# asharakeh/pod_compare

Measured on AMD Instinct MI355X. Metric: images/sec (BayesOD+MC-dropout, 1280x720), higher is better.
Workload: dtype f32 (convolutions: every fp32 product from 2-way f16 splits of the power-of-two-scaled fp32 operands, 3 partial products, fp32 accumulate; closer to fp64 than the fp32 MFMA: profiles/r05_f16_split_numerics.txt)

## Files before the change

include/pod_mi355x.h:

```cpp
#ifndef POD_MI355X_H
#define POD_MI355X_H

#include <stddef.h>
#include <stdint.h>

#ifdef __cplusplus
extern "C" {
#endif

#define POD_ABI_VERSION 18
#define POD_MAX_LEVELS 8
#define POD_MAX_CLASSES 16
#define POD_MAX_RUNS 64
#define POD_MAX_TOPK 2048
#define POD_MAX_PROP_SAMPLES 1024
#define POD_MAX_CLS_SAMPLES 64
#define POD_MAX_CANDIDATES 8192
#define POD_MAX_DETECTIONS 128
#define POD_COCO_MAX_IOU 16
#define POD_COCO_MAX_REC 128
#define POD_COCO_MAX_AREA 4
#define POD_COCO_MAX_MAXDET 4
#define POD_COCO_MAX_KEEP 128
#define POD_COCO_LDS_GT 64
// ... 280 lines not shown
int pod_resize_coeffs(int32_t in_size, int32_t out_size, int32_t* bounds, int32_t* coeffs);
int pod_resize_frame_u8(const uint8_t* src, int32_t in_h, int32_t in_w, int64_t row_stride, const int32_t* xbounds, const int32_t* xcoeffs,
                        int32_t xk, const int32_t* ybounds, const int32_t* ycoeffs, int32_t yk, uint8_t* dst, int32_t out_h, int32_t out_w,
                        int32_t flip_channels, pod_stream_t stream);

int pod_label_anchors(const float* anchors, int32_t R, const float* gt_boxes, const int32_t* gt_classes, const int32_t* gt_off,
                      int32_t n_images, int32_t n_gt, int32_t num_classes, float iou_low, float iou_high, int32_t* labels,
                      int32_t* matched_gt, int32_t* num_pos, uint32_t* scratch, pod_stream_t stream);

typedef struct PodLevelGrad {
    float* cls;  float* cls_var;  float* delta;  float* reg_var;
} PodLevelGrad;
int64_t pod_train_loss_partials(const PodConfig* cfg, const PodLevel* levels);
int pod_train_loss(const PodConfig* cfg, const PodLevel* levels, const PodLevelGrad* grads, const int32_t* labels,
                   const int32_t* matched_gt, const float* gt_boxes, int32_t n_gt, const float* anchors, int32_t R,
                   float alpha, float gamma, float smooth_l1_beta, const float* eps_cls, float* eps_out, const float* w,
                   double* partials, double* sums, pod_stream_t stream);

int64_t pod_conv3x3_wgrad_partials(const int32_t* level_hw, int32_t n_levels, int32_t copies, int32_t C, int32_t K, int32_t Kpad);
int pod_conv3x3_wgrad(const float* x, const float* dy, const int32_t* level_hw, int32_t n_levels, int32_t copies, int32_t C, int32_t K,
                      int32_t Kpad, const float* x_amax, const float* dy_amax, float* dW, float* db, float* partials, pod_stream_t stream);
int pod_relu_dropout_backward(const float* out, const float* d_out, float* d_z, int64_t n, float p, float* dz_amax, pod_stream_t stream);

int64_t pod_conv1x1_wgrad_partials(int64_t pixels, int32_t C, int32_t K);
int pod_conv1x1_wgrad(const float* x, const float* dy, int64_t pixels, int32_t C, int32_t K, const float* x_amax, const float* dy_amax, float* dW,
                      float* db, float* partials, pod_stream_t stream);
int pod_col2im3x3s2_cl(const float* dcols, const float* gate, const float* add, float* dx, int32_t H, int32_t W, int32_t C, float* dx_amax,
                       pod_stream_t stream);
int pod_upsample2_sum_cl(const float* d_child, int32_t h, int32_t w, const float* add, float* d_top, int32_t C, float* d_top_amax, pod_stream_t stream);


#define POD_C1_RELU 1
#define POD_C1_RESIDUAL_UP2 2
int64_t pod_conv1x1_filter_split_bytes(int32_t Cout, int32_t Cin);
int pod_conv1x1_filter_split(const float* weight, void* Ws, int32_t Cout, int32_t Cin, pod_stream_t stream);
int pod_reduce_partials(const float* partials, int32_t n_splits, int64_t split_stride, const float* bias, const float* residual, float* y,
                        int64_t n, int32_t Cout, int32_t relu, float* out_amax, pod_stream_t stream);
int pod_conv1x1_split(const float* x, float* y, const void* Ws, const float* bias, const float* residual, int32_t H_out, int32_t W_out,
                      int32_t H_in, int32_t W_in, int32_t stride, int32_t Cin, int32_t Cout, int32_t flags, int32_t n_splits, float* partials,
                      int32_t waves, const float* in_amax, float* out_amax, pod_stream_t stream);

typedef struct PodWorkspace {
    const float* anchors;
    float* mean_cls;  float* mean_cls_var;  float* mean_delta;  float* mean_reg_var;
    uint64_t* cand_keys;  int32_t* cand_count;  uint64_t* maybe_bits;
    uint64_t* sel_keys;   int32_t* sel_count;
    uint64_t* cat_keys;   int32_t* cat_level;
    float* probs_dense;
    int32_t* n_total;     int32_t* cand_anchor_idx;  int32_t* cand_level;  int32_t* cand_class;
    float* cand_score;    float* cand_probs;  float* cand_delta;  float* cand_reg_var;  float* cand_anchor;
    float* cand_run_delta;
    float* boxes;  float* cov;
    int32_t* keep;  int32_t* n_keep;  void* nms_scratch;
    float* m_boxes;  float* m_cov;  float* m_scores;  int32_t* m_classes;  float* m_probs;
    int32_t n_capacity;  int32_t reserved;
} PodWorkspace;

#define POD_MODE_STANDARD_NMS 0
#define POD_MODE_BAYES_OD 1
#define POD_MODE_ANCHOR_STATISTICS 2

int pod_run_image(const PodConfig* cfg, const PodLevel* levels, const PodWorkspace* ws, int32_t mode,
                  int32_t box_merge_mode, int32_t cls_merge_mode, int32_t image_h, int32_t image_w,
                  int32_t out_h, int32_t out_w, const PodDetections* out, pod_stream_t stream);
int pod_run_image_part(const PodConfig* cfg, const PodLevel* levels, const PodWorkspace* ws, int32_t mode,
                  int32_t box_merge_mode, int32_t cls_merge_mode, int32_t image_h, int32_t image_w,
// ... 7 lines not shown
```

pod_compare_amd/conv1x1.py:

```python
from typing import Optional

import torch

from . import amax, hip


class Conv1x1:

    def __init__(self, weight: torch.Tensor, bias: Optional[torch.Tensor], stride: int = 1):
        assert weight.is_cuda and weight.dtype == torch.float32 and weight.dim() == 4 and tuple(weight.shape[2:]) == (1, 1)
        self.K, self.C, self.stride = int(weight.shape[0]), int(weight.shape[1]), int(stride)
        if self.C % 16 or self.K % 64 or self.stride not in (1, 2):
            raise ValueError("pod_conv1x1_split: Cin %% 16 == 0, Cout %% 64 == 0, stride 1 or 2 required, got Cin=%d Cout=%d stride=%d" % (self.C, self.K, self.stride))
        self.Ws = torch.empty(2 * self.K * self.C + 8, dtype=torch.int16, device=weight.device)
        hip.check(hip.load().pod_conv1x1_filter_split(weight.detach().reshape(self.K, self.C).contiguous().data_ptr(), self.Ws.data_ptr(), self.K, self.C,
                                                      hip.current_stream()), "pod_conv1x1_filter_split")
        self.bias = None if bias is None else bias.detach().to(torch.float32).contiguous().clone()

    @staticmethod
    def eligible(conv: Optional[torch.nn.Conv2d]) -> bool:
        return (conv is not None and tuple(conv.kernel_size) == (1, 1) and tuple(conv.padding) == (0, 0) and conv.groups == 1
                and tuple(conv.dilation) == (1, 1) and conv.stride[0] == conv.stride[1] and conv.stride[0] in (1, 2)
                and conv.in_channels % 16 == 0 and conv.out_channels % 64 == 0)

    def out_hw(self, h: int, w: int):
        return ((h - 1) // self.stride + 1, (w - 1) // self.stride + 1)

    def splits_for(self, p_out: int, simds: int = 1024) -> int:
        tiles = ((p_out + 63) // 64) * (self.K // 64)
        nks = self.C // 16
        out_mb = p_out * self.K * 4 / 1e6
        step = 0.38
        best, best_t = 1, (nks // self.auto_waves(tiles, nks)) * step
        for s in (2, 4, 8, 16):
            if nks % s or nks // s < 4 or tiles * s > simds:
                continue
            t = (nks // s // self.auto_waves(tiles * s, nks // s)) * step + 3.0 + (s + 1) * out_mb / 4.0
            if t < best_t:
                best, best_t = s, t
        return best

    @staticmethod
    def auto_waves(tiles: int, per_split: int) -> int:
        waves = 1
        while waves < 4 and per_split % (waves * 4) == 0 and per_split // (waves * 2) >= 8 and tiles * waves * 2 <= 1024:
            waves *= 2
        return waves

    def __call__(self, x: torch.Tensor, h: int, w: int, relu: bool = False, residual: Optional[torch.Tensor] = None,
                 n_splits: Optional[int] = None, waves: int = 0, out: Optional[torch.Tensor] = None, residual_up2: bool = False) -> torch.Tensor:
        assert x.is_cuda and x.dtype == torch.float32 and x.is_contiguous() and tuple(x.shape) == (h * w, self.C)
        ho, wo = self.out_hw(h, w)
        y = torch.empty((ho * wo, self.K), dtype=torch.float32, device=x.device) if out is None else out
        assert y.is_contiguous() and tuple(y.shape) == (ho * wo, self.K) and y.dtype == torch.float32
        s = self.splits_for(ho * wo) if n_splits is None else int(n_splits)
        if residual is not None and residual_up2:
            hr, wr = (ho + 1) // 2, (wo + 1) // 2
            assert residual.is_contiguous() and tuple(residual.shape) == (hr * wr, self.K) and residual.dtype == torch.float32
            if s > 1:
                residual = residual.view(hr, wr, self.K).repeat_interleave(2, 0).repeat_interleave(2, 1)[:ho, :wo].reshape(ho * wo, self.K).contiguous()
                residual_up2 = False
        else:
            residual_up2 = False
        if residual is not None and not residual_up2:
            assert residual.is_contiguous() and tuple(residual.shape) == tuple(y.shape) and residual.dtype == torch.float32
        partials = torch.empty((s, ho * wo, self.K), dtype=torch.float32, device=x.device) if s > 1 else None
        hip.check(hip.load().pod_conv1x1_split(x.data_ptr(), y.data_ptr(), self.Ws.data_ptr(), hip.ptr(self.bias), hip.ptr(residual), ho, wo, h, w, self.stride,
                                               self.C, self.K, (1 if relu else 0) | (2 if residual_up2 else 0), s, hip.ptr(partials), int(waves), amax.of(x).data_ptr(), amax.produced(y).data_ptr(),
                                               hip.current_stream()), "pod_conv1x1_split")
        return y


class Stem7x7:

    def __init__(self, weight: torch.Tensor, bias: Optional[torch.Tensor]):
        assert weight.is_cuda and weight.dtype == torch.float32 and tuple(weight.shape) == (64, 3, 7, 7)
        self.Ws = torch.empty(2 * 64 * 192 + 8, dtype=torch.int16, device=weight.device)
        self._bounds = {}
        hip.check(hip.load().pod_stem7x7_filter_split(weight.detach().contiguous().data_ptr(), self.Ws.data_ptr(), hip.current_stream()), "pod_stem7x7_filter_split")
        self.bias = None if bias is None else bias.detach().to(torch.float32).contiguous().clone()

    @staticmethod
    def eligible(conv: Optional[torch.nn.Conv2d]) -> bool:
        return (conv is not None and tuple(conv.weight.shape) == (64, 3, 7, 7) and tuple(conv.stride) == (2, 2) and tuple(conv.padding) == (3, 3)
                and conv.groups == 1 and tuple(conv.dilation) == (1, 1))

    def __call__(self, x: torch.Tensor, relu: bool = True, mean: Optional[torch.Tensor] = None, std: Optional[torch.Tensor] = None,
                 padded_hw: Optional[tuple] = None):
        assert x.is_cuda and x.dtype in (torch.float32, torch.uint8) and x.is_contiguous() and x.numel() == 3 * x.shape[-2] * x.shape[-1]
        hi, wi = int(x.shape[-2]), int(x.shape[-1])
        h, w = (hi, wi) if padded_hw is None else (int(padded_hw[0]), int(padded_hw[1]))
        assert (mean is None) == (std is None) and h >= hi and w >= wi
        if mean is not None:
            assert mean.is_cuda and std.is_cuda and mean.dtype == std.dtype == torch.float32 and mean.numel() == std.numel() == 3 and mean.is_contiguous() and std.is_contiguous()
        ho, wo = (h - 1) // 2 + 1, (w - 1) // 2 + 1
        y = torch.empty((ho * wo, 64), dtype=torch.float32, device=x.device)
        bound = self._input_bound(x, mean, std)
        hip.check(hip.load().pod_stem7x7_split(x.data_ptr(), 1 if x.dtype == torch.uint8 else 0, hi, wi, hip.ptr(mean), hip.ptr(std), y.data_ptr(), self.Ws.data_ptr(),
                                               hip.ptr(self.bias), h, w, 1 if relu else 0, bound.data_ptr(), amax.produced(y).data_ptr(),
                                               hip.current_stream()), "pod_stem7x7_split")
        return y, ho, wo
# ... 53 lines not shown
```

pod_compare_amd/csrc/k13_conv1x1_split.hip:

```cpp
#include "pod_split_gemm.h"

#ifdef POD_C1_TRACE
static __device__ long long g_c1_trace[8192 * 4];
static __device__ long long g_c1_cycles[8192 * 4];
#define C1_STAMP(k)                                                                                   \
    do {                                                                                              \
        const unsigned wg_ = blockIdx.y * gridDim.x + blockIdx.x;                                     \
        if (threadIdx.x == 0 && wg_ < 8192) {                                                         \
            g_c1_trace[wg_ * 4 + (k)] = wall_clock64();                                               \
            g_c1_cycles[wg_ * 4 + (k)] = clock64();                                                   \
        }                                                                                             \
    } while (0)
#else
#define C1_STAMP(k)
#endif

namespace pod {

struct C1Params {
    const float* x;
    float* y;
    const uint16_t* Ws;
    const float* in_amax;
    float* out_amax;
    const float* bias;
    const float* residual;
    int32_t P_out, W_out, W_in, stride, Cin, Cout, relu;
    int32_t res_up2, W_res;
    int32_t n_pt, n_ct;
    int32_t ks_per_split;
    int64_t split_stride;
};

__global__ void __launch_bounds__(256) k_conv1x1_filter_split(const float* __restrict__ w, uint16_t* __restrict__ Ws, const float* __restrict__ amax, int32_t Cout,
                                                              int32_t Cin) {
    const int64_t t = (int64_t)blockIdx.x * blockDim.x + threadIdx.x;
    if (t >= (int64_t)Cout * (Cin / 2)) return;
    const int k = (int)(t / (Cin / 2)), c = 2 * (int)(t % (Cin / 2));
    sg_store_filter_terms(Ws, Cin >> 4, k, c, w[(int64_t)k * Cin + c], w[(int64_t)k * Cin + c + 1], amax);
}

template <int NCB>
__global__ void __launch_bounds__(64) k_conv1x1_split(const C1Params P) {
    const int lane = threadIdx.x & 63, i32 = lane & 31, h = lane >> 5;
    const int xcd = blockIdx.x & 7, wi = (int)(blockIdx.x >> 3);
    const int tp = (wi / P.n_ct) * 8 + xcd, tc = wi % P.n_ct;
    if (tp >= P.n_pt) return;
    C1_STAMP(0);
    const int nks_all = P.Cin >> 4, ks0 = (int)blockIdx.y * P.ks_per_split, nks = P.ks_per_split;
    int pout[2], pin[2];
#pragma unroll
    for (int pb = 0; pb < 2; ++pb) {
        const int p = tp * 64 + pb * 32 + i32;
        pout[pb] = p < P.P_out ? p : -1;
        const int q = p < P.P_out ? p : 0;
        if (P.stride == 1) {
            pin[pb] = q;
        } else {
            const int oy = q / P.W_out, ox = q - oy * P.W_out;
            pin[pb] = (P.stride * oy) * P.W_in + P.stride * ox;
        }
    }
    const float* __restrict__ xa[2];
#pragma unroll
// ... 97 lines not shown
__device__ __forceinline__ void c1_epilogue(const C1Params& P, float* const lds_o, f32x16 (&acc)[2][2], int tp, int tc, int lane, float sx) {
    float* __restrict__ const yo = P.y + (int64_t)blockIdx.y * P.split_stride;
    const float* __restrict__ const res = P.residual;
    const bool final_pass = P.split_stride == 0;
    const int oc = lane & 15, op = lane >> 4;
    const int gp0 = tp * 64 + op;
    const int64_t e0 = (int64_t)gp0 * P.Cout + tc * 64 + 4 * oc;
    f32x4 r[16];
    if (final_pass && res && P.res_up2) {
        int oy = gp0 / P.W_out, ox = gp0 - oy * P.W_out;
#pragma unroll
        for (int j = 0; j < 16; ++j) {
            r[j] = (gp0 + 4 * j < P.P_out) ? *reinterpret_cast<const f32x4*>(res + ((int64_t)(oy >> 1) * P.W_res + (ox >> 1)) * P.Cout + tc * 64 + 4 * oc)
                                           : f32x4{0.f, 0.f, 0.f, 0.f};
            ox += 4;
            while (ox >= P.W_out) {
                ox -= P.W_out;
                ++oy;
            }
        }
    } else if (final_pass && res) {
#pragma unroll
        for (int j = 0; j < 16; ++j) r[j] = (gp0 + 4 * j < P.P_out) ? *reinterpret_cast<const f32x4*>(res + e0 + (int64_t)(4 * j) * P.Cout) : f32x4{0.f, 0.f, 0.f, 0.f};
    }
    f32x4 b4 = f32x4{0.f, 0.f, 0.f, 0.f};
    if (final_pass && P.bias) b4 = *reinterpret_cast<const f32x4*>(P.bias + tc * 64 + 4 * oc);
    sg_line_epilogue(lds_o, acc, lane, sg_inverse_scale(sx, P.Ws, (int64_t)P.Cout * P.Cin * 2), b4, final_pass && res ? r : nullptr, final_pass && P.relu,
                     final_pass ? P.out_amax : nullptr, [&](int j, int, float*& dst) __attribute__((always_inline)) {
                         dst = yo + e0 + (int64_t)(4 * j) * P.Cout;
                         return gp0 + 4 * j < P.P_out;
                     });
}

template <int NCB, int WAVES>
__global__ void __launch_bounds__(64 * WAVES, WAVES > 1 ? 1 : 2) k_conv1x1_split_lds(const C1Params P) {
    __shared__ __attribute__((aligned(16))) float lds_all[WAVES][2][64 * 32];
    const int wave = threadIdx.x >> 6;
    float (*const lds_a)[64 * 32] = lds_all[wave];
    const int lane = threadIdx.x & 63, i32 = lane & 31, h = lane >> 5;
    const int xcd = blockIdx.x & 7, wi = (int)(blockIdx.x >> 3);
    const int tp = (wi / P.n_ct) * 8 + xcd, tc = wi % P.n_ct;
    if (tp >= P.n_pt) return;
    C1_STAMP(0);
    const int nks_all = P.Cin >> 4, nks = P.ks_per_split / WAVES, ks0 = (int)blockIdx.y * P.ks_per_split + wave * nks;
    int32_t soff[8];
#pragma unroll
    for (int j = 0; j < 8; ++j) {
        const int pl = 8 * j + (lane >> 3), p = tp * 64 + pl;
        const int q = p < P.P_out ? p : 0;
        int pin = q;
        if (P.stride != 1) {
            const int oy = q / P.W_out, ox = q - oy * P.W_out;
            pin = (P.stride * oy) * P.W_in + P.stride * ox;
        }
        soff[j] = pin * P.Cin + ks0 * 16 + 4 * ((lane & 7) ^ ((pl >> 1) & 7));
    }
    const float* __restrict__ const xg = P.x;
    const int key = (i32 >> 1) & 7;
    const uint16_t* __restrict__ const wa = P.Ws + ((int64_t)(tc * NCB) * nks_all + ks0) * SG_KS_U16 + (h * 32 + i32) * 8;
    const int64_t w_cb = (int64_t)nks_all * SG_KS_U16;
    const float sx = sg_activation_scale(P.in_amax);

    f32x16 acc[NCB][2];
#pragma unroll
    for (int cb = 0; cb < NCB; ++cb)
#pragma unroll
        for (int pb = 0; pb < 2; ++pb)
#pragma unroll
// ... 15 lines not shown
        constexpr int t = decltype(t_t)::value;
        sg_kstep<false>(acc, wf[buf], sx, [&](int pb, int i) __attribute__((always_inline)) {
            const f32x4 a = *reinterpret_cast<const f32x4*>(&lds_a[b][(pb * 32 + i32) * 32 + 4 * ((4 * t + 2 * h + (i >> 1)) ^ key)]);
            return f32x2{a[2 * (i & 1)], a[2 * (i & 1) + 1]};
        });
    };
    stage_load(0);
    load_w(sg_ic<0>{}, 0);
    load_w(sg_ic<1>{}, 1);
    stage_write(0);
    if (npairs > 1) stage_load(1);
    C1_STAMP(1);
    auto trip = [&](auto self, auto r_t, int j0) __attribute__((always_inline)) -> void {
        constexpr int R = decltype(r_t)::value;
        if constexpr (R < 6) {
            const int j = j0 + R;
            if (j < nks) {
                if (j + 2 < nks) load_w(sg_ic<(R + 2) % 3>{}, j + 2);
                const int pair = j >> 1;
                step(sg_ic<R % 3>{}, sg_ic<R & 1>{}, pair & 1);
                if constexpr ((R & 1) == 1) {
                    if (pair + 1 < npairs) {
                        stage_write((pair + 1) & 1);
                        if (pair + 2 < npairs) stage_load(pair + 2);
                    }
                }
                self(self, sg_ic<R + 1>{}, j0);
            }
        }
    };
    for (int j0 = 0; j0 < nks; j0 += 6) trip(trip, sg_ic<0>{}, j0);
    C1_STAMP(2);

    if constexpr (WAVES > 1) {
        if (wave > 0) {
            float* o = &lds_a[0][0];
#pragma unroll
            for (int cb = 0; cb < NCB; ++cb)
#pragma unroll
                for (int pb = 0; pb < 2; ++pb)
#pragma unroll
                    for (int r = 0; r < 16; ++r) o[((cb * 2 + pb) * 16 + r) * 64 + lane] = acc[cb][pb][r];
        }
        __syncthreads();
        if (wave > 0) return;
#pragma unroll
        for (int w = 1; w < WAVES; ++w) {
            const float* o = &lds_all[w][0][0];
#pragma unroll
            for (int cb = 0; cb < NCB; ++cb)
#pragma unroll
                for (int pb = 0; pb < 2; ++pb)
#pragma unroll
                    for (int r = 0; r < 16; ++r) acc[cb][pb][r] += o[((cb * 2 + pb) * 16 + r) * 64 + lane];
        }
    }
    c1_epilogue(P, &lds_a[0][0], acc, tp, tc, lane, sx);
#ifdef POD_C1_TRACE
    __builtin_amdgcn_s_waitcnt(0);
    C1_STAMP(3);
#endif
}

__global__ void __launch_bounds__(256) k_conv1x1_reduce(const float* __restrict__ partials, int32_t n_splits, int64_t split_stride, const float* __restrict__ bias,
                                                        const float* __restrict__ residual, float* __restrict__ y, int64_t n4, int32_t Cout, int32_t relu,
                                                        float* __restrict__ out_amax) {
    const int64_t stride = (int64_t)gridDim.x * blockDim.x;
// ... 1 lines not shown
    for (int64_t i = (int64_t)blockIdx.x * blockDim.x + threadIdx.x; i < n4; i += stride) {
        const f32x4 v = sg_split_sum4(partials, 4 * i, n_splits, split_stride, bias, [&](int64_t e) { return (int)(e % Cout); }, residual, relu);
        *reinterpret_cast<f32x4*>(y + 4 * i) = v;
        lmax = wino_absmax4(lmax, v);
    }
    if (out_amax) wino_publish_amax_block(out_amax, lmax);
}

}

extern "C" int64_t pod_conv1x1_filter_split_bytes(int32_t Cout, int32_t Cin) {
    if (Cout < 32 || (Cout & 31) != 0 || Cin < 16 || (Cin & 15) != 0) return 0;
    return (int64_t)Cout * Cin * 4 + 16;
}

extern "C" int pod_conv1x1_filter_split(const float* weight, void* Ws, int32_t Cout, int32_t Cin, pod_stream_t stream) {
    if (!weight || !Ws || Cout < 32 || (Cout & 31) != 0 || Cin < 16 || (Cin & 15) != 0 || !pod_aligned(16, Ws)) return POD_E_INVALID;
    const int64_t n = (int64_t)Cout * (Cin / 2);
    return pod::sg_filter_prepare(weight, (int64_t)Cout * Cin, Ws, (int64_t)Cout * Cin * 2, (hipStream_t)stream, [&](const float* amax) {
        hipLaunchKernelGGL(pod::k_conv1x1_filter_split, dim3((unsigned)((n + 255) / 256)), dim3(256), 0, (hipStream_t)stream, weight, reinterpret_cast<uint16_t*>(Ws), amax,
                           Cout, Cin);
    });
}

extern "C" int pod_conv1x1_split(const float* x, float* y, const void* Ws, const float* bias, const float* residual, int32_t H_out, int32_t W_out, int32_t H_in,
                                 int32_t W_in, int32_t stride, int32_t Cin, int32_t Cout, int32_t flags, int32_t n_splits, float* partials, int32_t waves,
                                 const float* in_amax, float* out_amax, pod_stream_t stream) {
    if (!x || !y || !Ws || !in_amax || x == y || H_out < 1 || W_out < 1 || (stride != 1 && stride != 2) || Cin < 16 || (Cin & 15) != 0 || Cout < 64 || (Cout & 63) != 0)
        return POD_E_INVALID;
    if (H_in < (H_out - 1) * stride + 1 || W_in < (W_out - 1) * stride + 1 || (stride == 1 && (H_in != H_out || W_in != W_out))) return POD_E_INVALID;
    const int64_t P_out = (int64_t)H_out * W_out;
    if (P_out * (Cout > Cin ? Cout : Cin) >= ((int64_t)1 << 31) || (int64_t)H_in * W_in * Cin >= ((int64_t)1 << 31)) return POD_E_INVALID;
    const int nks = Cin / 16;
    if (n_splits < 1 || n_splits > 16 || nks % n_splits != 0 || (n_splits > 1 && !partials)) return POD_E_INVALID;
    const int res_up2 = (flags & POD_C1_RESIDUAL_UP2) ? 1 : 0, relu = flags & POD_C1_RELU;
    if (res_up2 && (!residual || n_splits > 1)) return POD_E_INVALID;
    if (waves < 0 || waves > 4 || waves == 3) return POD_E_INVALID;
    {
        const int per_split = nks / n_splits;
        if (waves == 0) {
            const int64_t tiles = ((P_out + 63) / 64) * (Cout / 64) * n_splits;
            waves = 1;
            while (waves < 4 && per_split % (waves * 4) == 0 && per_split / (waves * 2) >= 8 && tiles * waves * 2 <= 1024) waves *= 2;
        }
        if (waves > 1 && (per_split % (2 * waves) != 0)) return POD_E_INVALID;
    }
    if (!pod_aligned(16, x, y, Ws, bias, residual, partials) || !pod_aligned(4, in_amax, out_amax)) return POD_E_INVALID;
    pod::C1Params P;
    P.x = x; P.y = n_splits > 1 ? partials : y; P.Ws = reinterpret_cast<const uint16_t*>(Ws); P.bias = bias; P.residual = residual;
    P.in_amax = in_amax; P.out_amax = out_amax;
    P.P_out = (int32_t)P_out; P.W_out = W_out; P.W_in = W_in; P.stride = stride; P.Cin = Cin; P.Cout = Cout; P.relu = relu;
    P.res_up2 = res_up2; P.W_res = (W_out + 1) / 2;
    P.n_pt = (int32_t)((P_out + 63) / 64); P.n_ct = Cout / 64;
    P.ks_per_split = nks / n_splits;
    P.split_stride = n_splits > 1 ? P_out * Cout : 0;
    const int64_t grid = 8LL * ((P.n_pt + 7) / 8) * P.n_ct;
    if (grid > 0x7FFFFFFFLL) return POD_E_INVALID;
    if ((P.ks_per_split & 1) == 0 && waves == 4)
        hipLaunchKernelGGL((pod::k_conv1x1_split_lds<2, 4>), dim3((unsigned)grid, (unsigned)n_splits), dim3(256), 0, (hipStream_t)stream, P);
    else if ((P.ks_per_split & 1) == 0 && waves == 2)
        hipLaunchKernelGGL((pod::k_conv1x1_split_lds<2, 2>), dim3((unsigned)grid, (unsigned)n_splits), dim3(128), 0, (hipStream_t)stream, P);
    else if ((P.ks_per_split & 1) == 0)
        hipLaunchKernelGGL((pod::k_conv1x1_split_lds<2, 1>), dim3((unsigned)grid, (unsigned)n_splits), dim3(64), 0, (hipStream_t)stream, P);
    else
        hipLaunchKernelGGL((pod::k_conv1x1_split<2>), dim3((unsigned)grid, (unsigned)n_splits), dim3(64), 0, (hipStream_t)stream, P);
    POD_CHECK_LAUNCH();
    if (n_splits > 1) {
        const int64_t n4 = P_out * Cout / 4;
        hipLaunchKernelGGL(pod::k_conv1x1_reduce, dim3(pod_grid_stride_blocks(n4, 2048)), dim3(256), 0, (hipStream_t)stream, partials, n_splits, P_out * Cout, bias, residual, y, n4,
                           Cout, relu, out_amax);
        POD_CHECK_LAUNCH();
    }
    return POD_OK;
}

extern "C" int pod_reduce_partials(const float* partials, int32_t n_splits, int64_t split_stride, const float* bias, const float* residual, float* y, int64_t n,
                                   int32_t Cout, int32_t relu, float* out_amax, pod_stream_t stream) {
    if (!partials || !y || n_splits < 1 || n_splits > 16 || n < 0 || (n & 3) != 0 || Cout < 4 || (Cout & 3) != 0 || n % Cout != 0) return POD_E_INVALID;
    if (n_splits > 1 && (split_stride < n || (split_stride & 3) != 0)) return POD_E_INVALID;
    if (!pod_aligned(16, partials, y, bias, residual)) return POD_E_INVALID;
    if (n == 0) return POD_OK;
    hipLaunchKernelGGL(pod::k_conv1x1_reduce, dim3(pod_grid_stride_blocks(n / 4, 4096)), dim3(256), 0, (hipStream_t)stream, partials, n_splits, split_stride, bias, residual, y, n / 4,
                       Cout, relu, out_amax);
    POD_CHECK_LAUNCH();
    return POD_OK;
}


#ifdef POD_C1_TRACE
#include <algorithm>
#include <stdio.h>
#include <vector>
extern "C" int pod_c1_trace_dump(void) {
    static long long host[8192 * 4], cyc[8192 * 4];
    if (hipDeviceSynchronize() != hipSuccess) return POD_E_LAUNCH;
    if (hipMemcpyFromSymbol(host, HIP_SYMBOL(g_c1_trace), sizeof(host)) != hipSuccess) return POD_E_LAUNCH;
    if (hipMemcpyFromSymbol(cyc, HIP_SYMBOL(g_c1_cycles), sizeof(cyc)) != hipSuccess) return POD_E_LAUNCH;
    long long t0 = 0, t_end = 0;
    std::vector<long long> start, first, loop, epi, total, mhz;
    for (int i = 0; i < 8192; ++i)
// ... 23 lines not shown
```

pod_compare_amd/csrc/pod_split_gemm.h:

```cpp
#pragma once
#include <type_traits>
#include <utility>

#include "pod_device.h"

namespace pod {

typedef float f32x16 __attribute__((ext_vector_type(16)));
typedef float f32x2 __attribute__((ext_vector_type(2)));

typedef _Float16 wino_f16x2 __attribute__((ext_vector_type(2)));
typedef _Float16 wino_f16x8 __attribute__((ext_vector_type(8)));
__device__ __forceinline__ float wino_pow2_scale(float amax, int top) {
    const int E = (int)((__float_as_uint(amax) >> 23) & 0xFFu);
    int b = 254 + top - E;
    b = b < 1 ? 1 : b > 254 ? 254 : b;
    return __uint_as_float((uint32_t)b << 23);
}
__device__ __forceinline__ float wino_pow2_inverse(float s) {
    return __uint_as_float((254u << 23) - __float_as_uint(s));
}
__device__ __forceinline__ uint32_t wino_f16_pair_scaled(float lo, float hi, float s) {
    uint32_t w;
    asm("v_fma_mixlo_f16 %0, %1, %3, 0\n\tv_fma_mixhi_f16 %0, %2, %3, 0" : "=&v"(w) : "v"(lo), "v"(hi), "s"(s));
// ... 121 lines not shown

template <typename Where>
__device__ __forceinline__ void sg_line_epilogue(float* lds, const f32x16 (&acc)[2][2], int lane, float inv1, const f32x4& b4, const f32x4* r, bool relu, float* out_amax,
                                                 Where&& where) {
    const int i32 = lane & 31, h = lane >> 5, oc = lane & 15, op = lane >> 4;
    const f32x4 inv = f32x4{inv1, inv1, inv1, inv1};
    float lmax = 0.0f;
#pragma unroll
    for (int pb = 0; pb < 2; ++pb)
#pragma unroll
        for (int cb = 0; cb < 2; ++cb)
#pragma unroll
            for (int q = 0; q < 4; ++q) {
                const int pix = 32 * pb + i32, c = 8 * cb + 2 * q + h;
                *reinterpret_cast<f32x4*>(lds + pix * 64 + 4 * (c ^ (i32 & 15))) =
                    f32x4{acc[cb][pb][4 * q], acc[cb][pb][4 * q + 1], acc[cb][pb][4 * q + 2], acc[cb][pb][4 * q + 3]};
            }
#pragma unroll
    for (int j = 0; j < 16; ++j) {
        const int pix = 4 * j + op;
        float* dst;
        const bool inside = where(j, pix, dst);
        f32x4 v = __builtin_elementwise_fma(*reinterpret_cast<const f32x4*>(lds + pix * 64 + 4 * (oc ^ (pix & 15))), inv, b4);
        if (r) v += r[j];
        if (relu) wino_relu4(v);
        if (inside) {
            *reinterpret_cast<f32x4*>(dst) = v;
            lmax = wino_absmax4(lmax, v);
        }
    }
    if (out_amax) wino_publish_amax(out_amax, lmax);
}

template <typename T>
__global__ void __launch_bounds__(256) k_sg_filter_amax(const T* __restrict__ w, int64_t n, float* __restrict__ amax) {
    float m = 0.0f;
    for (int64_t i = (int64_t)blockIdx.x * blockDim.x + threadIdx.x; i < n; i += (int64_t)gridDim.x * blockDim.x) m = fmaxf(m, fabsf(w[i]));
    wino_publish_amax1(amax, m);
}
__device__ __forceinline__ void sg_store_filter_terms(uint16_t* __restrict__ Ws, int nks, int co, int k, float lo, float hi, const float* __restrict__ amax) {
    uint32_t terms[2];
    wino_f16_split2(lo, hi, wino_pow2_scale(*amax, SG_TOP), terms);
    const int cb = co >> 5, i32 = co & 31, ks = k >> 4, h = (k >> 3) & 1, e = k & 7;
#pragma unroll
    for (int term = 0; term < 2; ++term) {
        uint16_t* d = Ws + ((((int64_t)cb * nks + ks) * 2 + term) * 2 + h) * 256 + i32 * 8 + e;
        d[0] = (uint16_t)(terms[term] & 0xFFFFu);
        d[1] = (uint16_t)(terms[term] >> 16);
    }
}
template <typename LaunchSplit>
inline int sg_filter_prepare(const float* weight, int64_t n, void* Ws, int64_t n_terms, hipStream_t stream, LaunchSplit&& launch_split) {
    float* amax = reinterpret_cast<float*>(reinterpret_cast<uint16_t*>(Ws) + n_terms);
    if (hipMemsetAsync(amax, 0, 16, stream) != hipSuccess) return POD_E_LAUNCH;
    const int64_t blocks = (n + 255) / 256;
    hipLaunchKernelGGL(k_sg_filter_amax<float>, dim3((unsigned)(blocks < 256 ? blocks : 256)), dim3(256), 0, stream, weight, n, amax);
    POD_CHECK_LAUNCH();
    launch_split(amax);
    POD_CHECK_LAUNCH();
    return POD_OK;
}

}
```

pod_compare_amd/csrc/k12_wino_conv_split.hip:

```cpp
#include "pod_wino.h"

namespace pod {

typedef uint32_t vu32x4 __attribute__((ext_vector_type(4)));
constexpr int WINO_US_BYTES = 24 * 2 * 2 * 64 * 16;
constexpr int WINO_U_TOP = 14, WINO_V_TOP = 9;
constexpr int WINO_WAIT_VM24 = 0x4078;

__global__ void __launch_bounds__(256) k_wino_filter_amax(const float* __restrict__ w, float* __restrict__ amax, int32_t K, int32_t C, int32_t Kpad) {
    const int64_t t = (int64_t)blockIdx.x * blockDim.x + threadIdx.x;
    float m = 0.0f;
    if (t < (int64_t)Kpad * C) {
        float u[4][6];
        wino_filter_values(w, (int)(t / C), (int)(t % C), K, C, u);
#pragma unroll
        for (int i = 0; i < 24; ++i) m = fmaxf(m, fabsf(u[i / 6][i % 6]));
    }
    wino_publish_amax1(amax, m);
}
__global__ void __launch_bounds__(256) k_wino_filter_split(const float* __restrict__ w, uint16_t* __restrict__ Us, const float* __restrict__ amax,
                                                           int32_t K, int32_t C, int32_t Kpad) {
    const int64_t t = (int64_t)blockIdx.x * blockDim.x + threadIdx.x;
    if (t >= (int64_t)Kpad * C) return;
    const int k = (int)(t / C), c = (int)(t % C);
    float u[4][6];
    wino_filter_values(w, k, c, K, C, u);
    const float sc = wino_pow2_scale(*amax, WINO_U_TOP);
    const int nchunk = C / 16, ks = k >> 6, kb = (k >> 5) & 1, j32 = k & 31, ch = c >> 4, hh = (c >> 3) & 1, e = c & 7;
    uint16_t* dst = Us + (((int64_t)ks * nchunk + ch) * (int64_t)WINO_US_BYTES) / 2 + (hh * 32 + j32) * 8 + e;
#pragma unroll
    for (int a = 0; a < 4; ++a)
#pragma unroll
        for (int p = 0; p < 6; ++p) {
            const float x = u[a][p] * sc;
            const _Float16 h0 = (_Float16)x;
            const _Float16 h1 = (_Float16)(x - (float)h0);
            uint16_t* d = dst + (((a * 6 + p) * 2 + kb) * 2) * 512;
            d[0] = __builtin_bit_cast(uint16_t, h0);
            d[512] = __builtin_bit_cast(uint16_t, h1);
        }
// ... 212 lines not shown
    };
    const int last = nchunk - 1, last_s = last >> 1;
    const int sc1 = last_s < 1 ? last_s : 1;
#pragma unroll
    for (int r = 0; r < 3; ++r) wino_mini_piece(r_rsrc, lds, a, 0, r, dmini[r]);
#pragma unroll
    for (int r = 0; r < 3; ++r) wino_mini_piece(r_rsrc, lds, a, 1, r, dmini[r]);
    WINO_STAMP(9);
    main_offsets();
    WINO_STAMP(10);
#pragma unroll
    for (int i = 0; i < 12; ++i) wino_patch_piece(r_rsrc, lds, a, 0, i, doff[i]);
#pragma unroll
    for (int i = 0; i < 6; ++i) wino_patch_piece(r_rsrc, lds + WINO_SB_FLOATS, a, sc1, i, doff[i]);
#pragma unroll
    for (int i = 0; i < 6; ++i) stage_load(i, sc1, 6 + i);
    WINO_STAMP(11);
    __builtin_amdgcn_s_waitcnt(WINO_WAIT_VM24);
    __builtin_amdgcn_s_barrier();
    WINO_STAMP(1);
    WINO_READ12(WINO_READ_MINI, 0);
    WINO_READS_LANDED();
    __builtin_amdgcn_sched_barrier(0);
    make_v(0);
    __builtin_amdgcn_sched_barrier(0);
    WINO_READ12(WINO_READ_MINI, 1);
    WINO_READS_LANDED();
    __builtin_amdgcn_sched_barrier(0);
    make_v(1);
    split_all();
    __builtin_amdgcn_sched_barrier(0);
    WINO_STAMP(2);
    const f32x16 zero16 = {0.f, 0.f, 0.f, 0.f, 0.f, 0.f, 0.f, 0.f, 0.f, 0.f, 0.f, 0.f, 0.f, 0.f, 0.f, 0.f};
    auto chunk = [&](auto mode_t, auto c16_t, auto par_t, int q) {
        constexpr int mode = decltype(mode_t)::value, c16 = decltype(c16_t)::value, par = decltype(par_t)::value;
        constexpr int n16 = c16 ^ 1, npar = c16 == 1 ? par ^ 1 : par;
        const int qn = q + 1 <= last ? q + 1 : last;
        const int ls0 = (q >> 1) + 2, ls = ls0 < last_s ? ls0 : last_s;
        wino_static_for([&](auto J) __attribute__((always_inline)) {
            constexpr int j = decltype(J)::value, p = j / 6, m = j % 6, kb = m & 1, prod = m >> 1;
            constexpr int sa = prod == 1 ? 1 : 0;
            constexpr int sb = prod == 0 ? 1 : 0;
            if constexpr (mode == 0 && prod == 0)
                acc[p * 2 + kb] = __builtin_amdgcn_mfma_f32_32x32x16_f16(__builtin_bit_cast(wino_f16x8, uP[p][kb * 2 + sa]), __builtin_bit_cast(wino_f16x8, Vb[p][sb]), zero16, 0, 0, 0);
            else
                acc[p * 2 + kb] = __builtin_amdgcn_mfma_f32_32x32x16_f16(__builtin_bit_cast(wino_f16x8, uP[p][kb * 2 + sa]), __builtin_bit_cast(wino_f16x8, Vb[p][sb]), acc[p * 2 + kb], 0, 0, 0);
            if constexpr (m < 4) { if (!(POD_WINO_ELIM & 2)) filter_piece(p + WINO_U_LEAD >= 6 ? qn : q, (p + WINO_U_LEAD) % 6, uP[(p + WINO_U_LEAD) % 6], m); }
            else if constexpr (m == 4) { if (!(POD_WINO_ELIM & 4)) stage_write(c16 == 0 ? par ^ 1 : par, p, c16 == 0 ? 6 + p : p); }
            if constexpr (p == 5 && m >= 4) {
                if (!(POD_WINO_ELIM & 4)) {
                    stage_load(3 * (m - 4), ls, 6 * c16 + 3 * (m - 4));
                    stage_load(3 * (m - 4) + 1, ls, 6 * c16 + 3 * (m - 4) + 1);
                    stage_load(3 * (m - 4) + 2, ls, 6 * c16 + 3 * (m - 4) + 2);
                }
            }
            if constexpr (mode != 0) {
                constexpr int u0 = j * N_UNITS / N_SLOTS, u1 = (j + 1) * N_UNITS / N_SLOTS;
                wino_static_for([&](auto K) __attribute__((always_inline)) {
                    unit(std::integral_constant<int, u0 + decltype(K)::value>{}, std::integral_constant<int, npar>{}, std::integral_constant<int, n16>{},
                         std::integral_constant<bool, mode == 2>{});
                }, std::make_integer_sequence<int, u1 - u0>{});
            }
            __builtin_amdgcn_sched_barrier(0);
        }, std::make_integer_sequence<int, N_SLOTS>{});
        __builtin_amdgcn_s_waitcnt(WINO_WAIT_LGKM0);
        __builtin_amdgcn_s_barrier();
        if constexpr (mode == 0) {
            if (q >= last) return;
            if constexpr (!(POD_WINO_ELIM & 1)) WINO_READ12(WINO_READ, npar, n16, 0);
            WINO_READS_LANDED();
            __builtin_amdgcn_sched_barrier(0);
            make_v(0);
            __builtin_amdgcn_sched_barrier(0);
            if constexpr (!(POD_WINO_ELIM & 1)) WINO_READ12(WINO_READ, npar, n16, 1);
            WINO_READS_LANDED();
            __builtin_amdgcn_sched_barrier(0);
            make_v(1);
            split_all();
            __builtin_amdgcn_sched_barrier(0);
            __builtin_amdgcn_s_barrier();
        }
    };
    using std::integral_constant;
    chunk(integral_constant<int, 0>{}, integral_constant<int, 0>{}, integral_constant<int, 0>{}, 0);
    if (nchunk > 1) chunk(integral_constant<int, 1>{}, integral_constant<int, 1>{}, integral_constant<int, 0>{}, 1);
    for (int base = 0;; base += 4) {
#define WINO_CHUNK(t)                                                                                                              \
    if (base + (t) >= nchunk) break;                                                                                               \
    chunk(integral_constant<int, 2>{}, integral_constant<int, (t) & 1>{}, integral_constant<int, ((t) >> 1) & 1>{}, base + (t));
        WINO_CHUNK(2) WINO_CHUNK(3) WINO_CHUNK(4) WINO_CHUNK(5)
#undef WINO_CHUNK
    }
    __syncthreads();
    WINO_STAMP(3);

    if (!wino_output_stage(acc, lds, a, i32, h)) return;
    const float inv = wino_pow2_inverse(sv) * wino_pow2_inverse(wino_pow2_scale(u_amax, WINO_U_TOP));
    const WinoStore S{set_out + (int64_t)blockIdx.y * P.split_out_stride, set_bias, set_out_amax, inv, set_offset, set_replicas, set_k_planes};
    const float lmax = S.k_planes > 0 ? wino_store_planes(P, B, S, lds, ks) : wino_store_channels_last(P, B, S, lds, ks);
    if (set_out_amax) wino_publish_amax_block(set_out_amax, lmax);
    WINO_STAMP_END();
}

}

#ifdef POD_TRACE
extern "C" int pod_wino_trace_dump_split(long long* host, int32_t n_workgroups) { return pod::wino_trace_dump(host, n_workgroups); }
#endif

extern "C" int64_t pod_wino_filter_split_bytes(int32_t K, int32_t C) {
    if (K < 1 || C < 16 || (C & 15) != 0) return 0;
    const int64_t Kpad = (K + 63) / 64 * 64;
    return Kpad / 64 * (C / 16) * (int64_t)pod::WINO_US_BYTES + 16;
}

extern "C" int pod_wino_filter_transform_split(const float* weight, void* Us, int32_t K, int32_t C, pod_stream_t stream) {
    if (!weight || !Us || K < 1 || C < 16 || (C & 15) != 0 || !pod_aligned(16, Us)) return POD_E_INVALID;
    const int32_t Kpad = (K + 63) / 64 * 64;
    const int64_t n = (int64_t)Kpad * C;
    float* amax = reinterpret_cast<float*>(reinterpret_cast<char*>(Us) + pod_wino_filter_split_bytes(K, C) - 16);
    if (hipMemsetAsync(amax, 0, 16, (hipStream_t)stream) != hipSuccess) return POD_E_LAUNCH;
    hipLaunchKernelGGL(pod::k_wino_filter_amax, dim3((unsigned)((n + 255) / 256)), dim3(256), 0, (hipStream_t)stream, weight, amax, K, C, Kpad);
    POD_CHECK_LAUNCH();
    hipLaunchKernelGGL(pod::k_wino_filter_split, dim3((unsigned)((n + 255) / 256)), dim3(256), 0, (hipStream_t)stream, weight,
// ... 40 lines not shown
```

Before: 139.1.

## Fuse split-K conv1x1 reduction into one launch via in-block wave groups

After: 136.8. 1.6% lower.

```diff
diff --git a/include/pod_mi355x.h b/include/pod_mi355x.h
--- a/include/pod_mi355x.h
+++ b/include/pod_mi355x.h
@@ -336,6 +336,7 @@
 
 #define POD_C1_RELU 1
 #define POD_C1_RESIDUAL_UP2 2
+#define POD_C1_ONE_LAUNCH 4
 int64_t pod_conv1x1_filter_split_bytes(int32_t Cout, int32_t Cin);
 int pod_conv1x1_filter_split(const float* weight, void* Ws, int32_t Cout, int32_t Cin, pod_stream_t stream);
 int pod_reduce_partials(const float* partials, int32_t n_splits, int64_t split_stride, const float* bias, const float* residual, float* y,
diff --git a/pod_compare_amd/conv1x1.py b/pod_compare_amd/conv1x1.py
--- a/pod_compare_amd/conv1x1.py
+++ b/pod_compare_amd/conv1x1.py
@@ -47,26 +47,34 @@
             waves *= 2
         return waves
 
+    @staticmethod
+    def one_launch(splits: int, waves: int, nks: int) -> bool:
+        return splits > 1 and splits * waves in (2, 4, 8) and (nks // splits) % (2 * waves) == 0
+
     def __call__(self, x: torch.Tensor, h: int, w: int, relu: bool = False, residual: Optional[torch.Tensor] = None,
-                 n_splits: Optional[int] = None, waves: int = 0, out: Optional[torch.Tensor] = None, residual_up2: bool = False) -> torch.Tensor:
+                 n_splits: Optional[int] = None, waves: int = 0, out: Optional[torch.Tensor] = None, residual_up2: bool = False,
+                 two_launches: bool = False) -> torch.Tensor:
         assert x.is_cuda and x.dtype == torch.float32 and x.is_contiguous() and tuple(x.shape) == (h * w, self.C)
         ho, wo = self.out_hw(h, w)
         y = torch.empty((ho * wo, self.K), dtype=torch.float32, device=x.device) if out is None else out
         assert y.is_contiguous() and tuple(y.shape) == (ho * wo, self.K) and y.dtype == torch.float32
         s = self.splits_for(ho * wo) if n_splits is None else int(n_splits)
+        nks = self.C // 16
+        wv = int(waves) if waves or nks % s else self.auto_waves(((ho * wo + 63) // 64) * (self.K // 64) * s, nks // s)
+        one = not two_launches and self.one_launch(s, wv, nks)
         if residual is not None and residual_up2:
             hr, wr = (ho + 1) // 2, (wo + 1) // 2
             assert residual.is_contiguous() and tuple(residual.shape) == (hr * wr, self.K) and residual.dtype == torch.float32
-            if s > 1:
+            if s > 1 and not one:
                 residual = residual.view(hr, wr, self.K).repeat_interleave(2, 0).repeat_interleave(2, 1)[:ho, :wo].reshape(ho * wo, self.K).contiguous()
                 residual_up2 = False
         else:
             residual_up2 = False
         if residual is not None and not residual_up2:
             assert residual.is_contiguous() and tuple(residual.shape) == tuple(y.shape) and residual.dtype == torch.float32
-        partials = torch.empty((s, ho * wo, self.K), dtype=torch.float32, device=x.device) if s > 1 else None
+        partials = torch.empty((s, ho * wo, self.K), dtype=torch.float32, device=x.device) if s > 1 and not one else None
         hip.check(hip.load().pod_conv1x1_split(x.data_ptr(), y.data_ptr(), self.Ws.data_ptr(), hip.ptr(self.bias), hip.ptr(residual), ho, wo, h, w, self.stride,
-                                               self.C, self.K, (1 if relu else 0) | (2 if residual_up2 else 0), s, hip.ptr(partials), int(waves), amax.of(x).data_ptr(), amax.produced(y).data_ptr(),
+                                               self.C, self.K, (1 if relu else 0) | (2 if residual_up2 else 0) | (4 if one else 0), s, hip.ptr(partials), wv, amax.of(x).data_ptr(), amax.produced(y).data_ptr(),
                                                hip.current_stream()), "pod_conv1x1_split")
         return y
 
diff --git a/pod_compare_amd/csrc/k13_conv1x1_split.hip b/pod_compare_amd/csrc/k13_conv1x1_split.hip
--- a/pod_compare_amd/csrc/k13_conv1x1_split.hip
+++ b/pod_compare_amd/csrc/k13_conv1x1_split.hip
@@ -30,6 +30,7 @@
     int32_t n_pt, n_ct;
     int32_t ks_per_split;
     int64_t split_stride;
+    int32_t group_waves;
 };
 
 __global__ void __launch_bounds__(256) k_conv1x1_filter_split(const float* __restrict__ w, uint16_t* __restrict__ Ws, const float* __restrict__ amax, int32_t Cout,
@@ -193,8 +194,58 @@
                      });
 }
 
-template <int NCB, int WAVES>
-__global__ void __launch_bounds__(64 * WAVES, WAVES > 1 ? 1 : 2) k_conv1x1_split_lds(const C1Params P) {
+template <int WAVES>
+__device__ __forceinline__ void c1_groups_epilogue(const C1Params& P, float* const lds, const f32x16 (&acc)[2][2], int tp, int tc, int wave, int lane, float sx) {
+    constexpr int NJ = 16 / WAVES;
+    sg_park_lines(lds + wave * 4096, acc, lane);
+    __syncthreads();
+    float* __restrict__ const yo = P.y;
+    const float* __restrict__ const res = P.residual;
+    const int oc = lane & 15, op = lane >> 4;
+    const int gp0 = tp * 64 + 4 * wave * NJ + op;
+    const int64_t e0 = (int64_t)gp0 * P.Cout + tc * 64 + 4 * oc;
+    f32x4 r[NJ];
+    if (res) {
+#pragma unroll
+        for (int jj = 0; jj < NJ; ++jj) {
+            const int gp = gp0 + 4 * jj;
+            int64_t re = e0 + (int64_t)(4 * jj) * P.Cout;
+            if (P.res_up2) {
+                const int oy = gp / P.W_out, ox = gp - oy * P.W_out;
+                re = ((int64_t)(oy >> 1) * P.W_res + (ox >> 1)) * P.Cout + tc * 64 + 4 * oc;
+            }
+            r[jj] = gp < P.P_out ? *reinterpret_cast<const f32x4*>(res + re) : f32x4{0.f, 0.f, 0.f, 0.f};
+        }
+    }
+    f32x4 b4 = f32x4{0.f, 0.f, 0.f, 0.f};
+    if (P.bias) b4 = *reinterpret_cast<const f32x4*>(P.bias + tc * 64 + 4 * oc);
+    const float inv1 = sg_inverse_scale(sx, P.Ws, (int64_t)P.Cout * P.Cin * 2);
+    const f32x4 inv = f32x4{inv1, inv1, inv1, inv1}, zero = f32x4{0.f, 0.f, 0.f, 0.f};
+    const int gw = P.group_waves;
+    float lmax = 0.0f;
+#pragma unroll
+    for (int jj = 0; jj < NJ; ++jj) {
+        const float* t = lds + sg_line_at(4 * (wave * NJ + jj) + op, oc);
+        f32x4 v = zero;
+        for (int g = 0; g < WAVES; g += gw) {
+            f32x4 a = *reinterpret_cast<const f32x4*>(t + g * 4096);
+            for (int i = 1; i < gw; ++i) a += *reinterpret_cast<const f32x4*>(t + (g + i) * 4096);
+            const f32x4 p = __builtin_elementwise_fma(a, inv, zero);
+            v = g == 0 ? p : v + p;
+        }
+        if (P.bias) v += b4;
+        if (res) v += r[jj];
+        if (P.relu) wino_relu4(v);
+        if (gp0 + 4 * jj < P.P_out) {
+            *reinterpret_cast<f32x4*>(yo + e0 + (int64_t)(4 * jj) * P.Cout) = v;
+            lmax = wino_absmax4(lmax, v);
+        }
+    }
+    if (P.out_amax) wino_publish_amax(P.out_amax, lmax);
+}
+
+template <int NCB, int WAVES, bool GROUPS = false>
+__global__ void __launch_bounds__(64 * WAVES, WAVES > 4 ? 2 : WAVES > 1 ? 1 : 2) k_conv1x1_split_lds(const C1Params P) {
     __shared__ __attribute__((aligned(16))) float lds_all[WAVES][2][64 * 32];
     const int wave = threadIdx.x >> 6;
     float (*const lds_a)[64 * 32] = lds_all[wave];
@@ -276,7 +327,10 @@
     for (int j0 = 0; j0 < nks; j0 += 6) trip(trip, sg_ic<0>{}, j0);
     C1_STAMP(2);
 
-    if constexpr (WAVES > 1) {
+    if constexpr (GROUPS) {
+        c1_groups_epilogue<WAVES>(P, &lds_all[0][0][0], acc, tp, tc, wave, lane, sx);
+        return;
+    } else if constexpr (WAVES > 1) {
         if (wave > 0) {
             float* o = &lds_a[0][0];
 #pragma unroll
@@ -344,9 +398,9 @@
     const int64_t P_out = (int64_t)H_out * W_out;
     if (P_out * (Cout > Cin ? Cout : Cin) >= ((int64_t)1 << 31) || (int64_t)H_in * W_in * Cin >= ((int64_t)1 << 31)) return POD_E_INVALID;
     const int nks = Cin / 16;
-    if (n_splits < 1 || n_splits > 16 || nks % n_splits != 0 || (n_splits > 1 && !partials)) return POD_E_INVALID;
+    if (n_splits < 1 || n_splits > 16 || nks % n_splits != 0 || (flags & ~(POD_C1_RELU | POD_C1_RESIDUAL_UP2 | POD_C1_ONE_LAUNCH))) return POD_E_INVALID;
     const int res_up2 = (flags & POD_C1_RESIDUAL_UP2) ? 1 : 0, relu = flags & POD_C1_RELU;
-    if (res_up2 && (!residual || n_splits > 1)) return POD_E_INVALID;
+    if (res_up2 && !residual) return POD_E_INVALID;
     if (waves < 0 || waves > 4 || waves == 3) return POD_E_INVALID;
     {
         const int per_split = nks / n_splits;
@@ -357,18 +411,28 @@
         }
         if (waves > 1 && (per_split % (2 * waves) != 0)) return POD_E_INVALID;
     }
+    const int total = n_splits * waves;
+    const bool in_launch = n_splits > 1 && (flags & POD_C1_ONE_LAUNCH) && (total == 2 || total == 4 || total == 8) && (nks / n_splits) % (2 * waves) == 0;
+    if (n_splits > 1 && !in_launch && (!partials || res_up2)) return POD_E_INVALID;
     if (!pod_aligned(16, x, y, Ws, bias, residual, partials) || !pod_aligned(4, in_amax, out_amax)) return POD_E_INVALID;
     pod::C1Params P;
-    P.x = x; P.y = n_splits > 1 ? partials : y; P.Ws = reinterpret_cast<const uint16_t*>(Ws); P.bias = bias; P.residual = residual;
+    P.x = x; P.y = n_splits > 1 && !in_launch ? partials : y; P.Ws = reinterpret_cast<const uint16_t*>(Ws); P.bias = bias; P.residual = residual;
     P.in_amax = in_amax; P.out_amax = out_amax;
     P.P_out = (int32_t)P_out; P.W_out = W_out; P.W_in = W_in; P.stride = stride; P.Cin = Cin; P.Cout = Cout; P.relu = relu;
     P.res_up2 = res_up2; P.W_res = (W_out + 1) / 2;
     P.n_pt = (int32_t)((P_out + 63) / 64); P.n_ct = Cout / 64;
-    P.ks_per_split = nks / n_splits;
-    P.split_stride = n_splits > 1 ? P_out * Cout : 0;
+    P.ks_per_split = in_launch ? nks : nks / n_splits;
+    P.group_waves = waves;
+    P.split_stride = n_splits > 1 && !in_launch ? P_out * Cout : 0;
     const int64_t grid = 8LL * ((P.n_pt + 7) / 8) * P.n_ct;
     if (grid > 0x7FFFFFFFLL) return POD_E_INVALID;
-    if ((P.ks_per_split & 1) == 0 && waves == 4)
+    if (in_launch && total == 8)
+        hipLaunchKernelGGL((pod::k_conv1x1_split_lds<2, 8, true>), dim3((unsigned)grid), dim3(512), 0, (hipStream_t)stream, P);
+    else if (in_launch && total == 4)
+        hipLaunchKernelGGL((pod::k_conv1x1_split_lds<2, 4, true>), dim3((unsigned)grid), dim3(256), 0, (hipStream_t)stream, P);
+    else if (in_launch)
+        hipLaunchKernelGGL((pod::k_conv1x1_split_lds<2, 2, true>), dim3((unsigned)grid), dim3(128), 0, (hipStream_t)stream, P);
+    else if ((P.ks_per_split & 1) == 0 && waves == 4)
         hipLaunchKernelGGL((pod::k_conv1x1_split_lds<2, 4>), dim3((unsigned)grid, (unsigned)n_splits), dim3(256), 0, (hipStream_t)stream, P);
     else if ((P.ks_per_split & 1) == 0 && waves == 2)
         hipLaunchKernelGGL((pod::k_conv1x1_split_lds<2, 2>), dim3((unsigned)grid, (unsigned)n_splits), dim3(128), 0, (hipStream_t)stream, P);
@@ -377,7 +441,7 @@
     else
         hipLaunchKernelGGL((pod::k_conv1x1_split<2>), dim3((unsigned)grid, (unsigned)n_splits), dim3(64), 0, (hipStream_t)stream, P);
     POD_CHECK_LAUNCH();
-    if (n_splits > 1) {
+    if (n_splits > 1 && !in_launch) {
         const int64_t n4 = P_out * Cout / 4;
         hipLaunchKernelGGL(pod::k_conv1x1_reduce, dim3(pod_grid_stride_blocks(n4, 2048)), dim3(256), 0, (hipStream_t)stream, partials, n_splits, P_out * Cout, bias, residual, y, n4,
                            Cout, relu, out_amax);
diff --git a/pod_compare_amd/csrc/pod_split_gemm.h b/pod_compare_amd/csrc/pod_split_gemm.h
--- a/pod_compare_amd/csrc/pod_split_gemm.h
+++ b/pod_compare_amd/csrc/pod_split_gemm.h
@@ -177,6 +177,21 @@
     if (out_amax) wino_publish_amax(out_amax, lmax);
 }
 
+__device__ __forceinline__ void sg_park_lines(float* lds, const f32x16 (&acc)[2][2], int lane) {
+    const int i32 = lane & 31, h = lane >> 5;
+#pragma unroll
+    for (int pb = 0; pb < 2; ++pb)
+#pragma unroll
+        for (int cb = 0; cb < 2; ++cb)
+#pragma unroll
+            for (int q = 0; q < 4; ++q) {
+                const int pix = 32 * pb + i32, c = 8 * cb + 2 * q + h;
+                *reinterpret_cast<f32x4*>(lds + pix * 64 + 4 * (c ^ (i32 & 15))) =
+                    f32x4{acc[cb][pb][4 * q], acc[cb][pb][4 * q + 1], acc[cb][pb][4 * q + 2], acc[cb][pb][4 * q + 3]};
+            }
+}
+__device__ __forceinline__ int sg_line_at(int pix, int oc) { return pix * 64 + 4 * (oc ^ (pix & 15)); }
+
 template <typename T>
 __global__ void __launch_bounds__(256) k_sg_filter_amax(const T* __restrict__ w, int64_t n, float* __restrict__ amax) {
     float m = 0.0f;
```

## Peel the final four Winograd chunks into tail forms that skip dead stage traffic

Applied to the files above, without the earlier changes.

New measurement: 136.7 before, 142.3 after, median of 6. 4.1% higher.

```diff
diff --git a/pod_compare_amd/csrc/k12_wino_conv_split.hip b/pod_compare_amd/csrc/k12_wino_conv_split.hip
--- a/pod_compare_amd/csrc/k12_wino_conv_split.hip
+++ b/pod_compare_amd/csrc/k12_wino_conv_split.hip
@@ -6,6 +6,7 @@
 constexpr int WINO_US_BYTES = 24 * 2 * 2 * 64 * 16;
 constexpr int WINO_U_TOP = 14, WINO_V_TOP = 9;
 constexpr int WINO_WAIT_VM24 = 0x4078;
+constexpr int WINO_TAIL_NO_LOAD = 1, WINO_TAIL_NO_PARK = 2, WINO_TAIL_LAST = 4;
 
 __global__ void __launch_bounds__(256) k_wino_filter_amax(const float* __restrict__ w, float* __restrict__ amax, int32_t K, int32_t C, int32_t Kpad) {
     const int64_t t = (int64_t)blockIdx.x * blockDim.x + threadIdx.x;
@@ -284,8 +285,10 @@
     __builtin_amdgcn_sched_barrier(0);
     WINO_STAMP(2);
     const f32x16 zero16 = {0.f, 0.f, 0.f, 0.f, 0.f, 0.f, 0.f, 0.f, 0.f, 0.f, 0.f, 0.f, 0.f, 0.f, 0.f, 0.f};
-    auto chunk = [&](auto mode_t, auto c16_t, auto par_t, int q) {
-        constexpr int mode = decltype(mode_t)::value, c16 = decltype(c16_t)::value, par = decltype(par_t)::value;
+    auto chunk = [&](auto mode_t, auto c16_t, auto par_t, auto tail_t, int q) {
+        constexpr int mode = decltype(mode_t)::value, c16 = decltype(c16_t)::value, par = decltype(par_t)::value, tail = decltype(tail_t)::value;
+        constexpr bool do_load = !(tail & WINO_TAIL_NO_LOAD), do_park = !(tail & WINO_TAIL_NO_PARK), is_last = (tail & WINO_TAIL_LAST) != 0;
+        static_assert((tail == 0 || mode == 2) && (!is_last || (!do_load && !do_park)), "tail forms are steady-state chunks; the last one has no stage traffic");
         constexpr int n16 = c16 ^ 1, npar = c16 == 1 ? par ^ 1 : par;
         const int qn = q + 1 <= last ? q + 1 : last;
         const int ls0 = (q >> 1) + 2, ls = ls0 < last_s ? ls0 : last_s;
@@ -297,9 +300,9 @@
                 acc[p * 2 + kb] = __builtin_amdgcn_mfma_f32_32x32x16_f16(__builtin_bit_cast(wino_f16x8, uP[p][kb * 2 + sa]), __builtin_bit_cast(wino_f16x8, Vb[p][sb]), zero16, 0, 0, 0);
             else
                 acc[p * 2 + kb] = __builtin_amdgcn_mfma_f32_32x32x16_f16(__builtin_bit_cast(wino_f16x8, uP[p][kb * 2 + sa]), __builtin_bit_cast(wino_f16x8, Vb[p][sb]), acc[p * 2 + kb], 0, 0, 0);
-            if constexpr (m < 4) { if (!(POD_WINO_ELIM & 2)) filter_piece(p + WINO_U_LEAD >= 6 ? qn : q, (p + WINO_U_LEAD) % 6, uP[(p + WINO_U_LEAD) % 6], m); }
-            else if constexpr (m == 4) { if (!(POD_WINO_ELIM & 4)) stage_write(c16 == 0 ? par ^ 1 : par, p, c16 == 0 ? 6 + p : p); }
-            if constexpr (p == 5 && m >= 4) {
+            if constexpr (m < 4 && (!is_last || p + WINO_U_LEAD < 6)) { if (!(POD_WINO_ELIM & 2)) filter_piece(p + WINO_U_LEAD >= 6 ? qn : q, (p + WINO_U_LEAD) % 6, uP[(p + WINO_U_LEAD) % 6], m); }
+            if constexpr (m == 4 && do_park) { if (!(POD_WINO_ELIM & 4)) stage_write(c16 == 0 ? par ^ 1 : par, p, c16 == 0 ? 6 + p : p); }
+            if constexpr (p == 5 && m >= 4 && do_load) {
                 if (!(POD_WINO_ELIM & 4)) {
                     stage_load(3 * (m - 4), ls, 6 * c16 + 3 * (m - 4));
                     stage_load(3 * (m - 4) + 1, ls, 6 * c16 + 3 * (m - 4) + 1);
@@ -309,14 +312,17 @@
             if constexpr (mode != 0) {
                 constexpr int u0 = j * N_UNITS / N_SLOTS, u1 = (j + 1) * N_UNITS / N_SLOTS;
                 wino_static_for([&](auto K) __attribute__((always_inline)) {
-                    unit(std::integral_constant<int, u0 + decltype(K)::value>{}, std::integral_constant<int, npar>{}, std::integral_constant<int, n16>{},
-                         std::integral_constant<bool, mode == 2>{});
+                    constexpr int u = u0 + decltype(K)::value;
+                    if constexpr (!is_last || (u >= 3 && u < 7))
+                        unit(std::integral_constant<int, u>{}, std::integral_constant<int, npar>{}, std::integral_constant<int, n16>{}, std::integral_constant<bool, mode == 2>{});
                 }, std::make_integer_sequence<int, u1 - u0>{});
             }
             __builtin_amdgcn_sched_barrier(0);
         }, std::make_integer_sequence<int, N_SLOTS>{});
-        __builtin_amdgcn_s_waitcnt(WINO_WAIT_LGKM0);
-        __builtin_amdgcn_s_barrier();
+        if constexpr (do_park) {
+            __builtin_amdgcn_s_waitcnt(WINO_WAIT_LGKM0);
+            __builtin_amdgcn_s_barrier();
+        }
         if constexpr (mode == 0) {
             if (q >= last) return;
             if constexpr (!(POD_WINO_ELIM & 1)) WINO_READ12(WINO_READ, npar, n16, 0);
@@ -334,14 +340,27 @@
         }
     };
     using std::integral_constant;
-    chunk(integral_constant<int, 0>{}, integral_constant<int, 0>{}, integral_constant<int, 0>{}, 0);
-    if (nchunk > 1) chunk(integral_constant<int, 1>{}, integral_constant<int, 1>{}, integral_constant<int, 0>{}, 1);
+    constexpr integral_constant<int, 0> I0{};
+    constexpr integral_constant<int, 1> I1{};
+    constexpr integral_constant<int, 2> I2{};
+    const bool peel = (nchunk & 3) == 0;
+    const int nloop = peel ? nchunk - 4 : nchunk;
+    chunk(I0, I0, I0, I0, 0);
+    if (nchunk > 1) chunk(I1, I1, I0, I0, 1);
     for (int base = 0;; base += 4) {
 #define WINO_CHUNK(t)                                                                                                              \
-    if (base + (t) >= nchunk) break;                                                                                               \
-    chunk(integral_constant<int, 2>{}, integral_constant<int, (t) & 1>{}, integral_constant<int, ((t) >> 1) & 1>{}, base + (t));
+    if (base + (t) >= nloop) break;                                                                                                \
+    chunk(I2, integral_constant<int, (t) & 1>{}, integral_constant<int, ((t) >> 1) & 1>{}, I0, base + (t));
         WINO_CHUNK(2) WINO_CHUNK(3) WINO_CHUNK(4) WINO_CHUNK(5)
 #undef WINO_CHUNK
+    }
+    if (peel) {
+        if (nchunk > 4) {
+            chunk(I2, I0, I0, integral_constant<int, WINO_TAIL_NO_LOAD>{}, nchunk - 4);
+            chunk(I2, I1, I0, integral_constant<int, WINO_TAIL_NO_LOAD | WINO_TAIL_NO_PARK>{}, nchunk - 3);
+        }
+        chunk(I2, I0, I1, integral_constant<int, WINO_TAIL_NO_LOAD | WINO_TAIL_NO_PARK>{}, nchunk - 2);
+        chunk(I2, I1, I1, integral_constant<int, WINO_TAIL_NO_LOAD | WINO_TAIL_NO_PARK | WINO_TAIL_LAST>{}, nchunk - 1);
     }
     __syncthreads();
     WINO_STAMP(3);
```
